# Boese0601/MagicDance

Measured on NVIDIA H100. Metric: denoise-steps/sec @512x512 50-step DDIM, higher is better.
Workload: dtype f16

## Files before the change

### magicdance_b200/csrc/gemm.cu

```cuda
#include <stdlib.h>

#include "common.cuh"

namespace mdb {

constexpr int kBM = 128;
constexpr int kBK = 64;

struct GemmKParams {
  CUtensorMap tmA;
  CUtensorMap tmA2;
  CUtensorMap tmB;
  __half* d;
  long long ldd;
  const float* bias;
  long long bias_batch_stride;
  const __half* residual;
  long long ldr;
  float* ws;
  int rows_per_batch;
  int m, n;
  int k_chunks;
  int k1_chunks;
  int chunks_per_split;
  int splits;
  int conv;
  int chunks_per_tap;
  int w, hw;
  int cs;
  int cluster_reduce;
  const float* ln_u;
  float ln_eps;
};

template <int BN, int STAGES>
struct GemmSmem {
  static constexpr int kABytes = kBM * kBK * 2;
  static constexpr int kBBytes = BN * kBK * 2;
  static constexpr int kStageBytes = kABytes + kBBytes;
  static constexpr int kTotal = STAGES * kStageBytes + 1024;
  static constexpr int kCtasPerSm = (kTotal <= 113 * 1024 && BN <= 128) ? 2 : 1;
};

__device__ __forceinline__ void epi_store_chunk(const GemmKParams& p, long long row, int col0, int ncols,
                                                float (&v)[32], const float* bias_chunk) {
  const __half* rp = (p.residual != nullptr) ? p.residual + row * p.ldr + col0 : nullptr;
  __half* dp = p.d + row * p.ldd + col0;
#pragma unroll
  for (int q = 0; q < 4; ++q) {
    if (q * 8 + 8 <= ncols) {
      float o[8];
#pragma unroll
      for (int e = 0; e < 8; ++e) o[e] = v[q * 8 + e];
      if (bias_chunk != nullptr) {
        const float4 b0 = *reinterpret_cast<const float4*>(bias_chunk + q * 8);
        const float4 b1 = *reinterpret_cast<const float4*>(bias_chunk + q * 8 + 4);
        o[0] += b0.x; o[1] += b0.y; o[2] += b0.z; o[3] += b0.w;
        o[4] += b1.x; o[5] += b1.y; o[6] += b1.z; o[7] += b1.w;
      }
      if (rp != nullptr) {
        const uint4 r4 = *reinterpret_cast<const uint4*>(rp + q * 8);
        const __half2* h2 = reinterpret_cast<const __half2*>(&r4);
#pragma unroll
        for (int e = 0; e < 4; ++e) {
          const float2 f = __half22float2(h2[e]);
          o[2 * e] += f.x;
          o[2 * e + 1] += f.y;
        }
      }
      uint4 o4;
      o4.x = pack_half2(o[0], o[1]);
      o4.y = pack_half2(o[2], o[3]);
      o4.z = pack_half2(o[4], o[5]);
      o4.w = pack_half2(o[6], o[7]);
      *reinterpret_cast<uint4*>(dp + q * 8) = o4;
    } else if (q * 8 < ncols) {
#pragma unroll
      for (int e = 0; e < 8; ++e) {
        const int j = q * 8 + e;
        if (j < ncols) {
          float x = v[j];
          if (bias_chunk != nullptr) x += bias_chunk[j];
          if (rp != nullptr) x += __half2float(rp[j]);
          dp[j] = __float2half_rn(x);
        }
      }
    }
  }
}

template <int BN, bool GEGLU, int kStages>
__global__ void __launch_bounds__(kWsThreads, (GemmSmem<BN, kStages>::kCtasPerSm))
    gemm_tc_kernel(const __grid_constant__ GemmKParams p) {
  using S = GemmSmem<BN, kStages>;
  extern __shared__ uint8_t smem_raw[];
  __shared__ __align__(8) uint64_t full_bar[kStages];
  __shared__ __align__(8) uint64_t empty_bar[kStages];
  __shared__ __align__(16) float s_bias[BN];
  __shared__ __align__(16) float s_lnu[BN];
  __shared__ float2 s_ln[kBM];

  uint8_t* smem = align1024(smem_raw);
  const int warp = threadIdx.x >> 5;
  const int lane = threadIdx.x & 31;
  const int m0 = blockIdx.x * kBM;
  const int n0 = blockIdx.y * BN;
  const int split = blockIdx.z;
  const int kc_begin = split * p.chunks_per_split;
  const int kc_end = min(p.k_chunks, kc_begin + p.chunks_per_split);
  const int n_iter = kc_end - kc_begin;
  constexpr int kRedLd = BN + 4;
  static_assert(kBM * kRedLd * 4 <= kStages * S::kStageBytes, "the accumulator tile must fit in the operand ring");
  const bool ln = p.ln_u != nullptr;

  pdl_launch_dependents();
  if (warp == kProducerWarp && lane == 0) {
    tma_prefetch_desc(&p.tmA);
    tma_prefetch_desc(&p.tmB);
    ring_init<kStages>(full_bar, empty_bar, 1);
    fence_barrier_init();
  }
  const bool bias_in_smem = (p.bias != nullptr) && (p.bias_batch_stride == 0) && !p.cluster_reduce;
  if (bias_in_smem && warp < kProducerWarp) {
    for (int j = threadIdx.x; j < BN; j += kConsumers) s_bias[j] = (n0 + j < p.n) ? p.bias[n0 + j] : 0.f;
  }
  if (ln && warp < kProducerWarp) {
    for (int j = threadIdx.x; j < BN; j += kConsumers) s_lnu[j] = (n0 + j < p.n) ? p.ln_u[n0 + j] : 0.f;
  }
  __syncthreads();
  pdl_wait();

  if (warp == kProducerWarp) {
    if (lane == 0 && n_iter > 0) {
      int b0 = 0, y0 = 0, x0 = 0;
      if (p.conv) {
        b0 = m0 / p.hw;
        y0 = (p.hw >= kBM) ? (m0 % p.hw) / p.w : 0;
        x0 = (p.hw >= kBM) ? (m0 % p.hw) % p.w : 0;
      }
      for (int it = 0; it < n_iter; ++it) {
        const int s = ring_acquire<kStages>(empty_bar, it);
        uint8_t* sa = smem + s * S::kStageBytes;
        uint8_t* sb = sa + S::kABytes;
        const int kc = kc_begin + it;
        mbar_expect_tx(&full_bar[s], S::kStageBytes);
        if (p.conv) {
          const int tap = kc / p.chunks_per_tap;
          const int cc = kc - tap * p.chunks_per_tap;
          const int kh = tap / 3, kw = tap - kh * 3;
          tma_load_4d(sa, &p.tmA, &full_bar[s], cc * kBK, p.cs * x0 + kw - 1, p.cs * y0 + kh - 1, b0);
        } else if (kc < p.k1_chunks) {
          tma_load_2d(sa, &p.tmA, &full_bar[s], kc * kBK, m0);
        } else {
          tma_load_2d(sa, &p.tmA2, &full_bar[s], (kc - p.k1_chunks) * kBK, m0);
        }
        tma_load_2d(sb, &p.tmB, &full_bar[s], kc * kBK, n0);
      }
    }
  } else {
    const int wg = warp >> 2;
    const int tid = threadIdx.x;
    float acc[BN / 2];
#pragma unroll
    for (int i = 0; i < BN / 2; ++i) acc[i] = 0.f;
    const int ln_row = tid >> 1, ln_half = tid & 1;
    float pivot = 0.f, ls0 = 0.f, ls1 = 0.f, lq0 = 0.f, lq1 = 0.f;
    for (int it = 0; it < n_iter; ++it) {
      const int s = ring_wait_full<kStages>(full_bar, it);
      const uint32_t a_addr = smem_u32(smem + s * S::kStageBytes);
      const uint64_t da = wgmma_desc_k_sw128(a_addr + wg * (64 * 128));
      const uint64_t db = wgmma_desc_k_sw128(a_addr + S::kABytes);
      wgmma_fence();
#pragma unroll
      for (int k = 0; k < kBK / 16; ++k) wgmma_ss<BN>(acc, da + 2 * k, db + 2 * k, 1u);
      wgmma_commit();
      if (ln) {
        const uint32_t arow = a_addr + (ln_row >> 3) * 1024 + (ln_row & 7) * 128;
        if (it == 0) {
          uint32_t w0;
          asm volatile("ld.shared.b32 %0, [%1];" : "=r"(w0) : "r"(arow + ((0 ^ (ln_row & 7)) << 4)));
          pivot = __low2float(*reinterpret_cast<const __half2*>(&w0));
        }
#pragma unroll
// ... 57 lines not shown
            if (ch * 32 + j < BN) {
              const float4 f = *reinterpret_cast<const float4*>(rrow + ch * 32 + j);
              v[j] = f.x; v[j + 1] = f.y; v[j + 2] = f.z; v[j + 3] = f.w;
            } else {
              v[j] = v[j + 1] = v[j + 2] = v[j + 3] = 0.f;
            }
          }
          if (ln) {
#pragma unroll
            for (int j = 0; j < 32; ++j)
              if (ch * 32 + j < BN) v[j] = lnst.y * fmaf(-lnst.x, s_lnu[ch * 32 + j], v[j]);
          }
          const int ncols = min(min(32, BN - ch * 32), p.n - col0);
          if (p.splits > 1) {
            if (row_ok) {
              float* wp = p.ws + (static_cast<long long>(split) * p.m + row) * p.n + col0;
#pragma unroll
              for (int j = 0; j < 32; j += 4) {
                if (j + 4 <= ncols && (p.n & 3) == 0) {
                  *reinterpret_cast<float4*>(wp + j) = make_float4(v[j], v[j + 1], v[j + 2], v[j + 3]);
                } else {
#pragma unroll
                  for (int e = 0; e < 4; ++e)
                    if (j + e < ncols) wp[j + e] = v[j + e];
                }
              }
            }
          } else if (row_ok) {
            const float* bias_chunk = nullptr;
            if (bias_in_smem) {
              bias_chunk = s_bias + ch * 32;
            } else if (p.bias != nullptr) {
              const long long brow = (p.bias_batch_stride != 0) ? (row / p.rows_per_batch) : 0;
              bias_chunk = p.bias + brow * p.bias_batch_stride + col0;
            }
            epi_store_chunk(p, row, col0, ncols, v, bias_chunk);
          }
        }
      }
    } else {
      const long long brow = (p.bias_batch_stride != 0) ? (row / p.rows_per_batch) : 0;
#pragma unroll 1
      for (int pr = half; pr < BN / 64; pr += 2) {
        const int col0 = n0 + pr * 64;
        if (col0 >= p.n) break;
        if (row_ok) {
          const float* bp = bias_in_smem ? (s_bias + pr * 64)
                                         : ((p.bias != nullptr) ? p.bias + brow * p.bias_batch_stride + col0 : nullptr);
          const float* rv = rrow + pr * 64;
          uint4* d4 = reinterpret_cast<uint4*>(p.d + row * p.ldd + (col0 >> 1));
#pragma unroll
          for (int q = 0; q < 4; ++q) {
            float o[8];
#pragma unroll
            for (int e = 0; e < 8; ++e) {
              const int j = q * 8 + e;
              float a = rv[j];
              float gt = rv[32 + j];
              if (bp != nullptr) {
                a += bp[j];
                gt += bp[32 + j];
              }
              o[e] = a * gelu_erf_f(gt);
            }
            uint4 o4;
            o4.x = pack_half2(o[0], o[1]);
            o4.y = pack_half2(o[2], o[3]);
            o4.z = pack_half2(o[4], o[5]);
            o4.w = pack_half2(o[6], o[7]);
// ... 18 lines not shown
          const int item = threadIdx.x + q * kWsThreads;
          if (item < R * groups) {
            const int rl = item / groups, cgp = item - rl * groups;
            const long long row = static_cast<long long>(m0) + static_cast<int>(crank) * R + rl;
            const int col0 = n0 + cgp * 8;
            if (row < p.m && col0 + 8 <= p.n) rpre[q] = *reinterpret_cast<const uint4*>(p.residual + row * p.ldr + col0);
          }
        }
      }
      cluster_sync_all();
      const uint32_t red_base = smem_u32(smem);
#pragma unroll 1
      for (int it_ = 0; it_ * kWsThreads < R * groups; ++it_) {
        const int item = threadIdx.x + it_ * kWsThreads;
        if (item >= R * groups) break;
        const int rl = item / groups, cgp = item - rl * groups;
        const int rt = static_cast<int>(crank) * R + rl;
        const long long row = static_cast<long long>(m0) + rt;
        const int col0 = n0 + cgp * 8;
        if (row >= p.m || col0 >= p.n) continue;
        const uint32_t off = red_base + static_cast<uint32_t>((rt * kRedLd + cgp * 8) * 4);
        float o[8];
#pragma unroll
        for (int e = 0; e < 8; ++e) o[e] = 0.f;
        for (int pr = 0; pr < S_; ++pr) {
          const uint32_t ra = dsmem_map(off, static_cast<uint32_t>(pr));
          const float4 a = dsmem_ld_f4(ra), b = dsmem_ld_f4(ra + 16);
          o[0] += a.x; o[1] += a.y; o[2] += a.z; o[3] += a.w;
          o[4] += b.x; o[5] += b.y; o[6] += b.z; o[7] += b.w;
        }
        const int ncols = min(8, p.n - col0);
        const long long brow = (p.bias_batch_stride != 0) ? (row / p.rows_per_batch) : 0;
        if (p.bias != nullptr) {
          const float* bp = p.bias + brow * p.bias_batch_stride + col0;
          for (int e = 0; e < ncols; ++e) o[e] += bp[e];
        }
        if (ncols == 8) {
          if (p.residual != nullptr) {
            uint4 r4 = make_uint4(0, 0, 0, 0);
            if (it_ < kMaxItems) {
#pragma unroll
              for (int q = 0; q < kMaxItems; ++q)
                if (q == it_) r4 = rpre[q];
            } else {
              r4 = *reinterpret_cast<const uint4*>(p.residual + row * p.ldr + col0);
            }
            const __half2* h2 = reinterpret_cast<const __half2*>(&r4);
#pragma unroll
            for (int e = 0; e < 4; ++e) {
              const float2 f = __half22float2(h2[e]);
              o[2 * e] += f.x;
              o[2 * e + 1] += f.y;
            }
          }
          uint4 o4;
          o4.x = pack_half2(o[0], o[1]);
          o4.y = pack_half2(o[2], o[3]);
          o4.z = pack_half2(o[4], o[5]);
          o4.w = pack_half2(o[6], o[7]);
          *reinterpret_cast<uint4*>(p.d + row * p.ldd + col0) = o4;
        } else {
          for (int e = 0; e < ncols; ++e) {
            float x = o[e];
            if (p.residual != nullptr) x += __half2float(p.residual[row * p.ldr + col0 + e]);
            p.d[row * p.ldd + col0 + e] = __float2half_rn(x);
          }
        }
      }
      cluster_sync_all();
    }
  }

}

__global__ void splitk_finalize_kernel(GemmKParams p) {
  pdl_launch_dependents();
  pdl_wait();
  const long long slab = static_cast<long long>(p.m) * p.n;
  if ((p.n & 3) == 0) {
    const long long total4 = slab >> 2;
    for (long long i = static_cast<long long>(blockIdx.x) * blockDim.x + threadIdx.x; i < total4;
         i += static_cast<long long>(gridDim.x) * blockDim.x) {
      const long long e = i << 2;
      const long long row = e / p.n;
      const int col = static_cast<int>(e - row * p.n);
      float4 a = *reinterpret_cast<const float4*>(p.ws + e);
      for (int s = 1; s < p.splits; ++s) {
        const float4 b = *reinterpret_cast<const float4*>(p.ws + s * slab + e);
        a.x += b.x; a.y += b.y; a.z += b.z; a.w += b.w;
      }
      if (p.bias != nullptr) {
        const long long brow = (p.bias_batch_stride != 0) ? (row / p.rows_per_batch) : 0;
        const float* bp = p.bias + brow * p.bias_batch_stride + col;
        a.x += bp[0]; a.y += bp[1]; a.z += bp[2]; a.w += bp[3];
      }
      if (p.residual != nullptr) {
        const __half2* rp = reinterpret_cast<const __half2*>(p.residual + row * p.ldr + col);
        const float2 r0 = __half22float2(rp[0]), r1 = __half22float2(rp[1]);
        a.x += r0.x; a.y += r0.y; a.z += r1.x; a.w += r1.y;
      }
      uint2 o;
      o.x = pack_half2(a.x, a.y);
      o.y = pack_half2(a.z, a.w);
      *reinterpret_cast<uint2*>(p.d + row * p.ldd + col) = o;
    }
    return;
  }
  for (long long i = static_cast<long long>(blockIdx.x) * blockDim.x + threadIdx.x; i < slab;
       i += static_cast<long long>(gridDim.x) * blockDim.x) {
    const long long row = i / p.n;
    const int col = static_cast<int>(i - row * p.n);
    float v = 0.f;
    for (int s = 0; s < p.splits; ++s) v += p.ws[s * slab + i];
    if (p.bias != nullptr) {
      const long long brow = (p.bias_batch_stride != 0) ? (row / p.rows_per_batch) : 0;
      v += p.bias[brow * p.bias_batch_stride + col];
    }
    if (p.residual != nullptr) v += __half2float(p.residual[row * p.ldr + col]);
    p.d[row * p.ldd + col] = __float2half_rn(v);
  }
}

int pixel_box(int ho, int wo, int cs, int rows, bool fwd, uint32_t box[4]) {
  const int hw = ho * wo;
  if (fwd ? wo > rows : wo >= rows) {
    if (wo % rows || (fwd && cs != 1)) return kBoxWideRows;
    box[1] = cs * rows; box[2] = 1; box[3] = 1;
  } else if (hw >= rows) {
    if (rows % wo || hw % rows) return kBoxRowsPerTile;
    box[1] = cs * wo; box[2] = cs * (rows / wo); box[3] = 1;
  } else {
    if (rows % hw) return kBoxImagesPerTile;
    box[1] = cs * wo; box[2] = cs * ho; box[3] = rows / hw;
  }
  box[0] = 64;
  return box[1] <= 256 && box[2] <= 256 ? kBoxOk : kBoxTooLarge;
}

static int g_pair_min_tiles = 128;
static int g_bn80_below = 100;
constexpr int kLongKChunks = 64;

template <int BN, bool GEGLU, int STAGES>
static int launch_gemm(const GemmKParams& kp, dim3 grid, cudaStream_t st) {
  const unsigned cluster_z = kp.cluster_reduce ? static_cast<unsigned>(kp.splits) : 1u;
  constexpr auto kern = gemm_tc_kernel<BN, GEGLU, STAGES>;
  constexpr int kSmem = GemmSmem<BN, STAGES>::kTotal;
  static_assert(kSmem <= 227 * 1024, "shared memory budget");
  if (int rc = set_max_dyn_smem<kern>(kSmem)) return rc;
  MDB_CHECK_CUDA(launch_pdl_cluster(kern, grid, dim3(kWsThreads), kSmem, st, cluster_z, kp));
  count_launch();
  return MDB_OK;
}

int get_gemm_tuning(int key) { return key == MDB_TUNE_GEMM_PAIR_MIN_TILES ? g_pair_min_tiles : g_bn80_below; }
void set_gemm_tuning(int key, int value) {
  if (key == MDB_TUNE_GEMM_PAIR_MIN_TILES) g_pair_min_tiles = value;
  else g_bn80_below = value;
}

}

using namespace mdb;

extern "C" int mdb_gemm_f16(const mdb_gemm_desc* g, mdb_stream_t stream) {
  MDB_REQUIRE(g != nullptr, "mdb_gemm_f16: null descriptor");
  MDB_REQUIRE(g->m > 0 && g->n > 0 && g->k > 0, "mdb_gemm_f16: bad shape m=%d n=%d k=%d", g->m, g->n, g->k);
  MDB_REQUIRE(g->k % kBK == 0, "mdb_gemm_f16: K=%d must be a multiple of 64", g->k);
  MDB_REQUIRE(g->a && g->b && g->d, "mdb_gemm_f16: null operand");
  cudaStream_t st = static_cast<cudaStream_t>(stream);
  const bool geglu = g->epilogue == MDB_EPI_GEGLU;
  GemmKParams kp;
  memset(&kp, 0, sizeof(kp));
  kp.d = static_cast<__half*>(g->d);
  kp.ldd = g->ldd;
  kp.bias = g->bias;
  kp.bias_batch_stride = g->bias_batch_stride;
  kp.rows_per_batch = g->rows_per_batch > 0 ? g->rows_per_batch : 1;
  kp.residual = static_cast<const __half*>(g->residual);
  kp.ldr = g->ldr;
  kp.m = g->m;
  kp.n = g->n;
  kp.k_chunks = g->k / kBK;
  kp.conv = g->conv;
  MDB_REQUIRE(g->ldd % 8 == 0 && (reinterpret_cast<uintptr_t>(g->d) & 15) == 0,
              "mdb_gemm_f16: D must be 16B aligned with ldd %% 8 == 0 (ldd=%lld)", (long long)g->ldd);
  if (g->bias) {
    MDB_REQUIRE((reinterpret_cast<uintptr_t>(g->bias) & 15) == 0 && g->bias_batch_stride % 4 == 0,
                "mdb_gemm_f16: bias must be 16B aligned with bias_batch_stride %% 4 == 0");
  }
  if (g->residual) {
    MDB_REQUIRE(g->ldr % 8 == 0 && (reinterpret_cast<uintptr_t>(g->residual) & 15) == 0,
                "mdb_gemm_f16: residual must be 16B aligned with ldr %% 8 == 0");
    MDB_REQUIRE(!geglu, "mdb_gemm_f16: residual is not supported with the GEGLU epilogue");
  }

  if (g->ln_u != nullptr) {
    MDB_REQUIRE(!geglu, "mdb_gemm_f16: LayerNorm fusion is not available with the GEGLU epilogue (N / 128 CTAs per row "
                        "block would each recompute the row statistics: measured slower than the LayerNorm kernel)");
    MDB_REQUIRE(!g->conv && g->a2 == nullptr && (reinterpret_cast<uintptr_t>(g->ln_u) & 15) == 0,
                "mdb_gemm_f16: LayerNorm fusion needs a plain single-source A whose K is the normalised width");
    kp.ln_u = g->ln_u;
    kp.ln_eps = g->ln_eps;
  }
  int rc;
  if (g->conv) {
    MDB_REQUIRE(g->a2 == nullptr, "mdb_gemm_f16: conv mode takes a single source");
    MDB_REQUIRE(g->c % kBK == 0 && g->k == 9 * g->c, "mdb_gemm_f16: conv needs c %% 64 == 0 and k == 9c (c=%d k=%d)",
                g->c, g->k);
    const int cs = g->conv == 2 ? 2 : 1;
    const int ho = (g->h - 1) / cs + 1, wo = (g->w - 1) / cs + 1;
    MDB_REQUIRE(g->m == g->nb * ho * wo, "mdb_gemm_f16: conv m != nb*ho*wo");
    const int hw = ho * wo;
    uint32_t box[4];
    const int why = pixel_box(ho, wo, cs, kBM, true, box);
    MDB_REQUIRE(why != kBoxWideRows, "mdb_gemm_f16: conv rows wider than 128 pixels need 128 | w and stride 1 (w=%d)", g->w);
    MDB_REQUIRE(why != kBoxRowsPerTile, "mdb_gemm_f16: conv tile needs w | 128 and 128 | h*w (output h=%d w=%d)", ho, wo);
    MDB_REQUIRE(why != kBoxImagesPerTile, "mdb_gemm_f16: conv tile needs h*w | 128 (output h=%d w=%d)", ho, wo);
    MDB_REQUIRE(why != kBoxTooLarge, "mdb_gemm_f16: conv TMA box too large");
    rc = tmap_nhwc(&kp.tmA, g->a, g->c, g->w, g->h, g->nb, g->c, box, cs);
    if (rc) return rc;
    kp.chunks_per_tap = g->c / kBK;
    kp.w = wo;
    kp.hw = hw;
    kp.cs = cs;
    kp.k1_chunks = kp.k_chunks;
  } else {
    const int k1 = g->a2 ? g->k1 : g->k;
    MDB_REQUIRE(k1 % kBK == 0 && k1 > 0 && k1 <= g->k, "mdb_gemm_f16: k1=%d must be a multiple of 64 within K", k1);
    rc = tmap_rows(&kp.tmA, g->a, k1, g->m, g->lda, kBK, kBM);
    if (rc) return rc;
    if (g->a2) {
      rc = tmap_rows(&kp.tmA2, g->a2, g->k - k1, g->m, g->lda2, kBK, kBM);
      if (rc) return rc;
    }
    kp.k1_chunks = k1 / kBK;
  }

  const int m_tiles = (g->m + kBM - 1) / kBM;
  bool pair = g->splits <= 1 && m_tiles >= 2 && g->n % 8 == 0 && g->ln_u == nullptr;
  int bn = 0;
  if (pair) {
    if (geglu) bn = (g->n % 256 == 0) ? 256 : 0;
    else if (g->n % 256 == 0) bn = 256;
    else if (g->n % 160 == 0) bn = 160;
    else bn = 128;
    const long long eq = (long long)m_tiles * ((g->n + bn - 1) / (bn ? bn : 1));
    if (bn == 0 || eq < (long long)g_pair_min_tiles || eq * kp.k_chunks < 16ll * g_pair_min_tiles) pair = false;
  }
  if (pair) {
  } else if (geglu) {
    MDB_REQUIRE(g->n % 128 == 0, "mdb_gemm_f16: GEGLU needs N %% 128 == 0 (N=%d)", g->n);
    bn = 128;
  } else if (g->n % 160 == 0) {
    const long long tiles160 = (long long)m_tiles * (g->n / 160) * (g->splits > 1 ? g->splits : 1);
    const bool wide_split = g->splits == 0 && kp.k_chunks >= kLongKChunks && tiles160 * 2 <= kNumSms;
    bn = (tiles160 < g_bn80_below && !wide_split) ? 80 : 160;
  } else {
    bn = 128;
  }
  rc = tmap_rows(&kp.tmB, g->b, g->k, g->n, g->ldb, kBK, bn);
  if (rc) return rc;

  int splits = g->splits > 1 ? g->splits : 1;
  if (g->ln_u != nullptr) splits = 1;
  if (g->splits == 0 && !geglu && !pair && g->ln_u == nullptr) {
    const long long tiles = (long long)m_tiles * ((g->n + bn - 1) / bn);
    if (tiles < 100)
      for (int c = 8; c >= 2; c >>= 1)
        if (tiles * c <= kNumSms && kp.k_chunks / c >= 16) {
          splits = c;
          break;
        }
  }
  if (splits > kp.k_chunks) splits = kp.k_chunks;
  if (geglu || pair) splits = 1;
  kp.chunks_per_split = (kp.k_chunks + splits - 1) / splits;
  splits = (kp.k_chunks + kp.chunks_per_split - 1) / kp.chunks_per_split;
  kp.splits = splits;
  kp.ws = g->splitk_ws;
  kp.cluster_reduce = (!geglu && (splits == 2 || splits == 4 || splits == 8)) ? 1 : 0;
  if (splits > 1 && !kp.cluster_reduce) {
    MDB_REQUIRE(g->splitk_ws != nullptr, "mdb_gemm_f16: splits > 1 needs splitk_ws");
  }

  dim3 grid(m_tiles, (g->n + bn - 1) / bn, splits);
  const bool deep = (long long)grid.x * grid.y * grid.z <= kNumSms && kp.chunks_per_split >= 12;
// ... 21 lines not shown
```

### magicdance_b200/engine.py

```python
from __future__ import annotations

from dataclasses import dataclass

import torch

from . import ops

UNET = "model.diffusion_model."
APPEARANCE = "appearance_control_model."
POSE = "pose_control_model."


@dataclass(frozen=True)
class NetConfig:
    in_channels: int = 4
    out_channels: int = 4
    hint_channels: int = 3
    model_channels: int = 320
    attention_resolutions: tuple = (4, 2, 1)
    num_res_blocks: int = 2
    channel_mult: tuple = (1, 2, 4, 4)
    num_heads: int = 8
    context_dim: int = 768

# ... 18 lines not shown
            inp.append(blk)
            chans.append(ch)
        if level != len(cfg.channel_mult) - 1:
            inp.append([("down", 0, ch, ch)])
            chans.append(ch)
            ds *= 2
    mid = [("res", 0, ch, ch), ("attn", 1, ch, ch), ("res", 2, ch, ch)]
    out = []
    for level, mult in list(enumerate(cfg.channel_mult))[::-1]:
        for i in range(cfg.num_res_blocks + 1):
            ich = chans.pop()
            blk = [("res", 0, ch + ich, mult * mc)]
            ch = mult * mc
            if ds in cfg.attention_resolutions:
                blk.append(("attn", len(blk), ch, ch))
            if level and i == cfg.num_res_blocks:
                blk.append(("up", len(blk), ch, ch))
                ds //= 2
            out.append(blk)
    return inp, mid, out


def _f16(t, device):
    return t.detach().to(device=device, dtype=torch.float16).contiguous()


def _f32(t, device):
    return t.detach().to(device=device, dtype=torch.float32).contiguous()


def pack_conv3x3(w, device):
    o, i, kh, kw = w.shape
    return _f16(w.detach().to(device).permute(0, 2, 3, 1).reshape(o, kh * kw * i), device)


def pack_conv1x1(w, device):
    return _f16(w.detach().reshape(w.shape[0], w.shape[1]), device)


def pack_geglu(w, b, device):
    n = w.shape[0] // 2
    idx = torch.arange(n).reshape(-1, 32)
    order = torch.cat([idx, idx + n], dim=1).reshape(-1)
    return _f16(w.detach()[order], device), _f32(b.detach()[order], device)


def fold_layernorm(w, gamma, beta, bias, device):
    w, gamma, beta = w.detach().to(device).float(), gamma.detach().to(device).float(), beta.detach().to(device).float()
    w_ln = (w * gamma[None, :]).to(torch.float16).contiguous()
    u = w_ln.float().sum(dim=1).contiguous()
    v = w @ beta
    if bias is not None:
        v = v + bias.detach().to(device).float()
    return w_ln, u, v.contiguous()


class ResW:
    pass


class AttnW:
    pass


class PackedNet:

# ... 8 lines not shown
        emb_w, emb_b, off = [], [], 0
        blocks = [(f"input_blocks.{i}.", b) for i, b in enumerate(self.inp)]
        blocks.append(("middle_block.", self.mid))
        if kind != "controlnet":
            blocks += [(f"output_blocks.{i}.", b) for i, b in enumerate(self.out)]
        for bp, blk in blocks:
            for kind_, j, cin, cout in blk:
                p = f"{bp}{j}."
                if kind_ == "conv_in":
                    self.layers[p] = (pack_conv3x3(g(p + "weight"), device), _f32(g(p + "bias"), device))
                elif kind_ == "res":
                    r = ResW()
                    r.cin, r.cout = cin, cout
                    r.gn1 = (_f32(g(p + "in_layers.0.weight"), device), _f32(g(p + "in_layers.0.bias"), device))
                    r.w1 = pack_conv3x3(g(p + "in_layers.2.weight"), device)
                    r.gn2 = (_f32(g(p + "out_layers.0.weight"), device), _f32(g(p + "out_layers.0.bias"), device))
                    r.w2 = pack_conv3x3(g(p + "out_layers.3.weight"), device)
                    r.b2 = _f32(g(p + "out_layers.3.bias"), device)
                    if (prefix + p + "skip_connection.weight") in sd:
                        r.skip_w = pack_conv1x1(g(p + "skip_connection.weight"), device)
                        r.skip_b = _f32(g(p + "skip_connection.bias"), device)
                    else:
                        r.skip_w = r.skip_b = None
                    emb_w.append(g(p + "emb_layers.1.weight").detach())
                    emb_b.append(g(p + "emb_layers.1.bias").detach() + g(p + "in_layers.2.bias").detach())
                    r.emb_off = off
                    off += cout
                    self.layers[p] = r
                elif kind_ == "attn":
                    self.layers[p] = self._pack_attn(g, p, cin, device)
                elif kind_ == "down":
                    self.layers[p] = (pack_conv3x3(g(p + "op.weight"), device), _f32(g(p + "op.bias"), device))
                elif kind_ == "up":
                    self.layers[p] = (pack_conv3x3(g(p + "conv.weight"), device), _f32(g(p + "conv.bias"), device))
        self.emb_w = _f16(torch.cat(emb_w, 0), device)
        self.emb_b = _f32(torch.cat(emb_b, 0), device)
        self.emb_total = off
        if kind == "unet":
            self.out_gn = (_f32(g("out.0.weight"), device), _f32(g("out.0.bias"), device))
            self.out_w, self.out_b = pack_conv3x3(g("out.2.weight"), device), _f32(g("out.2.bias"), device)
        if kind == "controlnet":
            self.hint = []
            for i in range(8):
                w = g(f"input_hint_block.{2 * i}.weight")
                self.hint.append((pack_conv3x3(w, device), _f32(g(f"input_hint_block.{2 * i}.bias"), device),
                                  w.shape[1], w.shape[0]))
            self.zero = []
            for i in range(len(self.inp)):
                self.zero.append((pack_conv1x1(g(f"zero_convs.{i}.0.weight"), device),
                                  _f32(g(f"zero_convs.{i}.0.bias"), device)))
            self.zero.append((pack_conv1x1(g("middle_block_out.0.weight"), device),
                              _f32(g("middle_block_out.0.bias"), device)))

    def _pack_attn(self, g, p, c, device):
        a = AttnW()
        a.c, a.heads, a.d = c, self.cfg.num_heads, c // self.cfg.num_heads
        a.gn = (_f32(g(p + "norm.weight"), device), _f32(g(p + "norm.bias"), device))
        a.pin_w, a.pin_b = pack_conv1x1(g(p + "proj_in.weight"), device), _f32(g(p + "proj_in.bias"), device)
        a.pout_w, a.pout_b = pack_conv1x1(g(p + "proj_out.weight"), device), _f32(g(p + "proj_out.bias"), device)
        t = p + "transformer_blocks.0."
        for i in (1, 3):
            setattr(a, f"ln{i}", (_f32(g(t + f"norm{i}.weight"), device), _f32(g(t + f"norm{i}.bias"), device)))
        a.wqk = _f16(torch.cat([g(t + "attn1.to_q.weight").detach(), g(t + "attn1.to_k.weight").detach()], 0), device)
        a.wv = _f16(g(t + "attn1.to_v.weight"), device)
        a.wo, a.bo = _f16(g(t + "attn1.to_out.0.weight"), device), _f32(g(t + "attn1.to_out.0.bias"), device)
        a.wq2_ln, a.q2_u, a.q2_v = fold_layernorm(g(t + "attn2.to_q.weight"), g(t + "norm2.weight"), g(t + "norm2.bias"),
                                                  None, device)
# ... 38 lines not shown

_warned_sizes = set()


def _igemm_ok(h, w, c):
    hw = h * w
    if c % 64:
        return False
    ok = ((128 % w == 0 and hw % 128 == 0) or w % 128 == 0) if hw >= 128 else (128 % hw == 0)
    if not ok and (h, w) not in _warned_sizes:
        _warned_sizes.add((h, w))
        import warnings
        warnings.warn(f"magicdance_b200: a {h}x{w} feature map does not tile into 128-pixel TMA boxes; its 3x3 convs take "
                      "the slower im2col + GEMM path (latents whose width divides 128 avoid this)", stacklevel=3)
    return ok


def conv3x3(x: Act, w, bias, *, cout, stride=1, residual=None, bias_batch_stride=0) -> Act:
    cin = x.c
    ho, wo = (x.h - 1) // stride + 1, (x.w - 1) // stride + 1
    tc = cout % 8 == 0 and cout >= 64 and cin % 64 == 0
    if tc and _igemm_ok(ho, wo, cin):
        y = ops.gemm(x.data, w, bias=bias, bias_batch_stride=bias_batch_stride, rows_per_batch=ho * wo,
                     residual=residual, conv=(x.b, x.h, x.w, cin), conv_stride=stride)
    elif tc:
        col = ops.im2col3x3(x.data, batch=x.b, h=x.h, w=x.w, c=cin, stride=stride)
        y = ops.gemm(col, w, bias=bias, bias_batch_stride=bias_batch_stride, rows_per_batch=ho * wo,
                     residual=residual)
    else:
        assert bias_batch_stride == 0
        y = ops.conv3x3_direct(x.data, w, bias, batch=x.b, h=x.h, w=x.w, cin=cin, cout=cout, stride=stride,
                               residual=residual)
    return Act(y, x.b, ho, wo)


class _BankComplete(Exception):
    """unwinds appearance_write as soon as the last norm1 state is in the bank"""


class DenoiseEngine:

    def __init__(self, state_dict, cfg: NetConfig | None = None, device="cuda"):
        ops.ensure_device()
        self.cfg = cfg or NetConfig()
        self.device = torch.device(device)
        self.unet = PackedNet(state_dict, UNET, self.cfg, "unet", self.device)
        self.appearance = PackedNet(state_dict, APPEARANCE, self.cfg, "appearance", self.device)
        self.pose = PackedNet(state_dict, POSE, self.cfg, "controlnet", self.device)
        self._ctx_cache = {}

    @classmethod
    def from_packed(cls, unet: "PackedNet", appearance: "PackedNet | None", pose: "PackedNet | None"):
        ops.ensure_device()
        self = cls.__new__(cls)
        first = unet or appearance or pose
        self.cfg, self.device = first.cfg, first.device
        self.unet, self.appearance, self.pose = unet, appearance, pose
        self._ctx_cache = {}
        return self

    def time_bias(self, net: PackedNet, t: torch.Tensor, rows=None):
        if t.shape[0] == 1:
            rows = 1
        e = ops.timestep_embedding(t, self.cfg.model_channels, rows)
        e = ops.skinny_linear(e, net.te0_w, net.te0_b, silu_out=True)
        e = ops.skinny_linear(e, net.te2_w, net.te2_b)
# ... 65 lines not shown
            k1, vt1, nb1, kvb1 = bank_kv
            kw = dict(k1=k1, vt1=vt1, n1=nb1, kv1_batches=kvb1, bank_batches=min(bank_batches, b))
        at = ops.attention(qk[:, :c], qk[:, c:], vt, n, heads=a.heads, d=a.d, batch=b, nq=n, **kw)
        h = ops.gemm(at, a.wo, bias=a.bo, residual=h)
        q2 = ops.gemm(h, a.wq2_ln, bias=a.q2_v, ln_u=a.q2_u, ln_eps=1e-5)
        kt, vtt, nt, kvb, ldv = ctx_kv
        at2 = ops.attention(q2, kt, vtt, nt, heads=a.heads, d=a.d, batch=b, nq=n, kv0_batches=kvb if kvb == b else 1,
                            ldv0_batch=ldv)
        h = ops.gemm(at2, a.wo2, bias=a.bo2, residual=h)
        n3 = ops.layernorm(h, *a.ln3)
        ff = ops.gemm(n3, a.wff1, bias=a.bff1, epilogue=ops.EPI_GEGLU)
        h = ops.gemm(ff, a.wff2, bias=a.bff2, residual=h)
        y = ops.gemm(h, a.pout_w, bias=a.pout_b, residual=x.data)
        return Act(y, x.b, x.h, x.w)

    def _run_block(self, net, bp, blk, x: Act, skip, emb_all, ctx_kvs, state):
        for kind, j, cin, cout in blk:
            p = f"{bp}{j}."
            lw = net.layers[p]
            if kind == "conv_in":
                x = conv3x3(x, lw[0], lw[1], cout=cout, residual=state.get("hint"))
            elif kind == "res":
                x = self._res(lw, x, skip, emb_all)
                skip = None
            elif kind == "attn":
                i = state["attn_i"]
                bank_kv = state["bank_kv"][i] if state.get("bank_kv") is not None else None
                x = self._transformer(lw, x, ctx_kvs[i], state["mode"], state.get("bank"), bank_kv,
                                      state.get("bank_batches", 0))
                state["attn_i"] = i + 1
            elif kind == "down":
                x = conv3x3(x, lw[0], lw[1], cout=cout, stride=2)
            elif kind == "up":
                up = ops.upsample2x(x.data, batch=x.b, h=x.h, w=x.w, c=x.c)
                x = conv3x3(Act(up, x.b, 2 * x.h, 2 * x.w), lw[0], lw[1], cout=cout)
        return x

    def _prep(self, x_nchw, context, copies=1):
        x = x_nchw.to(device=self.device, dtype=torch.float32)
        b, c, h, w = x.shape
        act = Act(ops.nchw_f32_to_nhwc_f16(x, copies=copies), copies * b, h, w)
        ctx16 = context.to(device=self.device, dtype=torch.float16).contiguous()
        return act, ctx16

    def appearance_write(self, ref_latent, t, context):
        net = self.appearance
        x, ctx16 = self._prep(ref_latent, context)
        ctx_kvs = self.context_kv(net, ctx16, context)
        emb_all = self.time_bias(net, t, x.b)
        n_total = len(net.attn_layers())
        state = {"mode": "write", "attn_i": 0, "bank": [], "bank_batches": n_total}
        hs = []
        try:
            for i, blk in enumerate(net.inp):
                x = self._run_block(net, f"input_blocks.{i}.", blk, x, None, emb_all, ctx_kvs, state)
                hs.append(x)
            x = self._run_block(net, "middle_block.", net.mid, x, None, emb_all, ctx_kvs, state)
            for i, blk in enumerate(net.out):
                x = self._run_block(net, f"output_blocks.{i}.", blk, x, hs.pop(), emb_all, ctx_kvs, state)
        except _BankComplete:
            pass
        return state["bank"]

    def attn_geometry(self, h, w):
        net = self.unet
        geo = []
        for blk in net.inp:
            for kind, _, _, cout in blk:
# ... 134 lines not shown
```

### magicdance_b200/ops.py

```python
from __future__ import annotations

import ctypes as C
import os

import torch

from . import _lib

EPI_NONE, EPI_GEGLU = 0, 1
SKINNY_MAX_ROWS = 16
_GEMM_DEBUG = os.environ.get("MDB_GEMM_DEBUG", "0") == "1"
TRACE = None


class tuning:
    _KEYS = {"pair_min_tiles": _lib.TUNE_GEMM_PAIR_MIN_TILES,
             "attn40_2q_min_ctas": _lib.TUNE_ATTN40_2Q_MIN_CTAS, "bn80_below": _lib.TUNE_GEMM_BN80_BELOW}

    def __init__(self, **kw):
        self.want = {self._KEYS[k]: int(v) for k, v in kw.items() if v is not None}

    def __enter__(self):
        lib = _lib.load()
        self.old = {k: int(lib.mdb_get_tuning(k)) for k in self.want}
        for k, v in self.want.items():
            _lib.check(lib.mdb_set_tuning(k, v), "set_tuning")
        return self

    def __exit__(self, *a):
        lib = _lib.load()
        for k, v in self.old.items():
            lib.mdb_set_tuning(k, v)


def _stream() -> int:
    return torch.cuda.current_stream().cuda_stream


def _ptr(t):
    return None if t is None else t.data_ptr()


# ... 35 lines not shown

    def __enter__(self):
        global _ws_tag
        self.prev, _ws_tag = _ws_tag, self.tag

    def __exit__(self, *a):
        global _ws_tag
        _ws_tag = self.prev


def current_lane():
    return _ws_tag


_ws_retired = []


def _workspace(key, numel, dtype, device, zero=False):
    k = (key, device, _ws_tag)
    t = _ws_cache.get(k)
    if t is None or t.numel() < numel or t.dtype != dtype:
        if t is not None:
            _ws_retired.append(t)
            numel = max(numel, 2 * t.numel())
        alloc = torch.zeros if zero else torch.empty
        t = alloc(max(numel, 1), dtype=dtype, device=device)
        _ws_cache[k] = t
    return t


def _gemm_m(a, conv, conv_stride, m):
    if conv is not None:
        nb, h, wd, _ = conv
        return nb * ((h - 1) // conv_stride + 1) * ((wd - 1) // conv_stride + 1)
    return a.shape[0] if m is None else m


def _fill_fwd_desc(g, a, w, a2, conv, conv_stride, m):
    n, k = w.shape
    if conv is not None:
        nb, h, wd, c = conv
        assert conv_stride in (1, 2) and a.is_contiguous() and a.numel() == nb * h * wd * c
        g.conv, g.nb, g.h, g.w, g.c = conv_stride, nb, h, wd, c
        g.a, g.lda, g.k1 = a.data_ptr(), c, k
    else:
        assert a.dim() == 2 and a.stride(1) == 1
        g.a, g.lda, g.k1 = a.data_ptr(), a.stride(0), a.shape[1]
        if a2 is not None:
            _chk(a2, torch.float16, "a2")
            assert a2.dim() == 2 and a2.stride(1) == 1 and a2.shape[0] == a.shape[0]
            g.a2, g.lda2 = a2.data_ptr(), a2.stride(0)
            assert a.shape[1] + a2.shape[1] == k
        else:
            assert a.shape[1] == k, (a.shape, w.shape)
    m = _gemm_m(a, conv, conv_stride, m)
    g.m, g.n, g.k = m, n, k
    return m, g.k1


def gemm(a, w, *, out=None, bias=None, bias_batch_stride=0, rows_per_batch=0, residual=None, epilogue=EPI_NONE,
         a2=None, conv=None, conv_stride=1, splits=0, m=None, ln_u=None, ln_eps=1e-5):
    lib = _lib.load()
    _chk(a, torch.float16, "a")
    _chk(w, torch.float16, "w")
    g = _lib.GemmDesc()
    n, k = w.shape
    m, _ = _fill_fwd_desc(g, a, w, a2, conv, conv_stride, m)
    n_out = n // 2 if epilogue == EPI_GEGLU else n
    if out is None:
        out = torch.empty((m, n_out), dtype=torch.float16, device=a.device)
    _chk(out, torch.float16, "out")
    assert out.dim() == 2 and out.stride(1) == 1 and out.shape[0] >= m and out.shape[1] == n_out, (out.shape, m, n_out)
    assert w.stride(1) == 1
    g.b, g.ldb = w.data_ptr(), w.stride(0)
    g.d, g.ldd = out.data_ptr(), out.stride(0)
    if bias is not None:
        _chk(bias, torch.float32, "bias")
        g.bias, g.bias_batch_stride, g.rows_per_batch = bias.data_ptr(), bias_batch_stride, rows_per_batch
    if residual is not None:
        _chk(residual, torch.float16, "residual")
        assert residual.dim() == 2 and residual.stride(1) == 1
        g.residual, g.ldr = residual.data_ptr(), residual.stride(0)
    g.epilogue = epilogue
    if ln_u is not None:
        _chk(ln_u, torch.float32, "ln_u")
        assert conv is None and a2 is None and ln_u.numel() == n and ln_u.is_contiguous()
        g.ln_u, g.ln_eps = ln_u.data_ptr(), float(ln_eps)
        splits = 1
    if TRACE is not None:
        TRACE.append((m, n, k, (tuple(conv) + (conv_stride,)) if conv is not None else None, epilogue, splits,
                      a2.shape[1] if a2 is not None else 0))
    if splits > 1:
        ws = _workspace("splitk", splits * m * n, torch.float32, a.device)
        g.splits, g.splitk_ws = splits, ws.data_ptr()
    else:
        g.splits = splits
    if _GEMM_DEBUG:
        import sys
        print(f"gemm m={m} n={n} k={k} conv={conv} epi={epilogue} splits={g.splits} a2={a2 is not None} lda={g.lda} "
              f"ldd={g.ldd} bias={bias is not None} bbs={g.bias_batch_stride} res={residual is not None}",
              file=sys.stderr, flush=True)
    _lib.check(lib.mdb_gemm_f16(C.byref(g), _stream()), "gemm_f16")
    if _GEMM_DEBUG:
        torch.cuda.synchronize()
    return out
# ... 757 lines not shown
```

Baseline: 89.92.

## Fuse nearest-2x upsample into the following 3x3 conv via four 2x2 phase convs

Replaces the separate upsample2x kernel plus a 3x3 conv on the upsampled map with a single implicit-GEMM over the low-resolution input. The weights are pre-summed into four 2x2 phase kernels, stacked along N. The epilogue scatters each phase's columns to the interleaved high-resolution output rows. This removes the upsampled intermediate's memory traffic and cuts the reduction length from 9c to 4c per output pixel. In exchange it adds per-element address arithmetic in the epilogue, strided output writes, and fp16 rounding of the summed weights.

```diff
diff --git a/magicdance_b200/csrc/gemm.cu b/magicdance_b200/csrc/gemm.cu
--- a/magicdance_b200/csrc/gemm.cu
+++ b/magicdance_b200/csrc/gemm.cu
@@ -28,6 +28,7 @@
   int chunks_per_tap;
   int w, hw;
   int cs;
+  int up_n;
   int cluster_reduce;
   const float* ln_u;
   float ln_eps;
@@ -42,10 +43,24 @@
   static constexpr int kCtasPerSm = (kTotal <= 113 * 1024 && BN <= 128) ? 2 : 1;
 };
 
+template <bool UP>
+__device__ __forceinline__ __half* d_at(const GemmKParams& p, long long row, int col) {
+  if (!UP) return p.d + row * p.ldd + col;
+  const int ph = col / p.up_n;
+  const long long img = row / p.hw;
+  const int r = static_cast<int>(row - img * p.hw);
+  const int y = r / p.w, x = r - y * p.w;
+  const long long orow = (img * (2 * (p.hw / p.w)) + 2 * y + (ph >> 1)) * (2 * p.w) + 2 * x + (ph & 1);
+  return p.d + orow * p.ldd + (col - ph * p.up_n);
+}
+template <bool UP>
+__device__ __forceinline__ int bias_col(const GemmKParams& p, int col) { return UP ? col % p.up_n : col; }
+
+template <bool UP>
 __device__ __forceinline__ void epi_store_chunk(const GemmKParams& p, long long row, int col0, int ncols,
                                                 float (&v)[32], const float* bias_chunk) {
   const __half* rp = (p.residual != nullptr) ? p.residual + row * p.ldr + col0 : nullptr;
-  __half* dp = p.d + row * p.ldd + col0;
+  __half* dp = d_at<UP>(p, row, col0);
 #pragma unroll
   for (int q = 0; q < 4; ++q) {
     if (q * 8 + 8 <= ncols) {
@@ -89,7 +104,7 @@
   }
 }
 
-template <int BN, bool GEGLU, int kStages>
+template <int BN, bool GEGLU, int kStages, bool UP>
 __global__ void __launch_bounds__(kWsThreads, (GemmSmem<BN, kStages>::kCtasPerSm))
     gemm_tc_kernel(const __grid_constant__ GemmKParams p) {
   using S = GemmSmem<BN, kStages>;
@@ -109,6 +124,9 @@
   const int kc_begin = split * p.chunks_per_split;
   const int kc_end = min(p.k_chunks, kc_begin + p.chunks_per_split);
   const int n_iter = kc_end - kc_begin;
+  const int phase = UP ? n0 / p.up_n : 0;
+  const int py = phase >> 1, px = phase & 1;
+  constexpr int kTaps = UP ? 2 : 3;
   constexpr int kRedLd = BN + 4;
   static_assert(kBM * kRedLd * 4 <= kStages * S::kStageBytes, "the accumulator tile must fit in the operand ring");
   const bool ln = p.ln_u != nullptr;
@@ -122,7 +140,7 @@
   }
   const bool bias_in_smem = (p.bias != nullptr) && (p.bias_batch_stride == 0) && !p.cluster_reduce;
   if (bias_in_smem && warp < kProducerWarp) {
-    for (int j = threadIdx.x; j < BN; j += kConsumers) s_bias[j] = (n0 + j < p.n) ? p.bias[n0 + j] : 0.f;
+    for (int j = threadIdx.x; j < BN; j += kConsumers) s_bias[j] = (n0 + j < p.n) ? p.bias[bias_col<UP>(p, n0 + j)] : 0.f;
   }
   if (ln && warp < kProducerWarp) {
     for (int j = threadIdx.x; j < BN; j += kConsumers) s_lnu[j] = (n0 + j < p.n) ? p.ln_u[n0 + j] : 0.f;
@@ -147,8 +165,8 @@
         if (p.conv) {
           const int tap = kc / p.chunks_per_tap;
           const int cc = kc - tap * p.chunks_per_tap;
-          const int kh = tap / 3, kw = tap - kh * 3;
-          tma_load_4d(sa, &p.tmA, &full_bar[s], cc * kBK, p.cs * x0 + kw - 1, p.cs * y0 + kh - 1, b0);
+          const int kh = tap / kTaps, kw = tap - kh * kTaps;
+          tma_load_4d(sa, &p.tmA, &full_bar[s], cc * kBK, p.cs * x0 + kw + px - 1, p.cs * y0 + kh + py - 1, b0);
         } else if (kc < p.k1_chunks) {
           tma_load_2d(sa, &p.tmA, &full_bar[s], kc * kBK, m0);
         } else {
@@ -272,9 +290,9 @@
               bias_chunk = s_bias + ch * 32;
             } else if (p.bias != nullptr) {
               const long long brow = (p.bias_batch_stride != 0) ? (row / p.rows_per_batch) : 0;
-              bias_chunk = p.bias + brow * p.bias_batch_stride + col0;
+              bias_chunk = p.bias + brow * p.bias_batch_stride + bias_col<UP>(p, col0);
             }
-            epi_store_chunk(p, row, col0, ncols, v, bias_chunk);
+            epi_store_chunk<UP>(p, row, col0, ncols, v, bias_chunk);
           }
         }
       }
@@ -359,7 +377,7 @@
         const int ncols = min(8, p.n - col0);
         const long long brow = (p.bias_batch_stride != 0) ? (row / p.rows_per_batch) : 0;
         if (p.bias != nullptr) {
-          const float* bp = p.bias + brow * p.bias_batch_stride + col0;
+          const float* bp = p.bias + brow * p.bias_batch_stride + bias_col<UP>(p, col0);
           for (int e = 0; e < ncols; ++e) o[e] += bp[e];
         }
         if (ncols == 8) {
@@ -385,12 +403,13 @@
           o4.y = pack_half2(o[2], o[3]);
           o4.z = pack_half2(o[4], o[5]);
           o4.w = pack_half2(o[6], o[7]);
-          *reinterpret_cast<uint4*>(p.d + row * p.ldd + col0) = o4;
+          *reinterpret_cast<uint4*>(d_at<UP>(p, row, col0)) = o4;
         } else {
+          __half* dp = d_at<UP>(p, row, col0);
           for (int e = 0; e < ncols; ++e) {
             float x = o[e];
             if (p.residual != nullptr) x += __half2float(p.residual[row * p.ldr + col0 + e]);
-            p.d[row * p.ldd + col0 + e] = __float2half_rn(x);
+            dp[e] = __float2half_rn(x);
           }
         }
       }
@@ -418,7 +437,7 @@
       }
       if (p.bias != nullptr) {
         const long long brow = (p.bias_batch_stride != 0) ? (row / p.rows_per_batch) : 0;
-        const float* bp = p.bias + brow * p.bias_batch_stride + col;
+        const float* bp = p.bias + brow * p.bias_batch_stride + (p.up_n ? bias_col<true>(p, col) : col);
         a.x += bp[0]; a.y += bp[1]; a.z += bp[2]; a.w += bp[3];
       }
       if (p.residual != nullptr) {
@@ -429,7 +448,7 @@
       uint2 o;
       o.x = pack_half2(a.x, a.y);
       o.y = pack_half2(a.z, a.w);
-      *reinterpret_cast<uint2*>(p.d + row * p.ldd + col) = o;
+      *reinterpret_cast<uint2*>(p.up_n ? d_at<true>(p, row, col) : d_at<false>(p, row, col)) = o;
     }
     return;
   }
@@ -441,10 +460,10 @@
     for (int s = 0; s < p.splits; ++s) v += p.ws[s * slab + i];
     if (p.bias != nullptr) {
       const long long brow = (p.bias_batch_stride != 0) ? (row / p.rows_per_batch) : 0;
-      v += p.bias[brow * p.bias_batch_stride + col];
+      v += p.bias[brow * p.bias_batch_stride + (p.up_n ? bias_col<true>(p, col) : col)];
     }
     if (p.residual != nullptr) v += __half2float(p.residual[row * p.ldr + col]);
-    p.d[row * p.ldd + col] = __float2half_rn(v);
+    *(p.up_n ? d_at<true>(p, row, col) : d_at<false>(p, row, col)) = __float2half_rn(v);
   }
 }
 
@@ -468,16 +487,24 @@
 static int g_bn80_below = 100;
 constexpr int kLongKChunks = 64;
 
-template <int BN, bool GEGLU, int STAGES>
-static int launch_gemm(const GemmKParams& kp, dim3 grid, cudaStream_t st) {
+template <int BN, bool GEGLU, int STAGES, bool UP>
+static int launch_gemm_t(const GemmKParams& kp, dim3 grid, cudaStream_t st) {
   const unsigned cluster_z = kp.cluster_reduce ? static_cast<unsigned>(kp.splits) : 1u;
-  constexpr auto kern = gemm_tc_kernel<BN, GEGLU, STAGES>;
+  constexpr auto kern = gemm_tc_kernel<BN, GEGLU, STAGES, UP>;
   constexpr int kSmem = GemmSmem<BN, STAGES>::kTotal;
   static_assert(kSmem <= 227 * 1024, "shared memory budget");
   if (int rc = set_max_dyn_smem<kern>(kSmem)) return rc;
   MDB_CHECK_CUDA(launch_pdl_cluster(kern, grid, dim3(kWsThreads), kSmem, st, cluster_z, kp));
   count_launch();
   return MDB_OK;
+}
+
+template <int BN, bool GEGLU, int STAGES>
+static int launch_gemm(const GemmKParams& kp, dim3 grid, cudaStream_t st) {
+  if constexpr (!GEGLU) {
+    if (kp.up_n) return launch_gemm_t<BN, false, STAGES, true>(kp, grid, st);
+  }
+  return launch_gemm_t<BN, GEGLU, STAGES, false>(kp, grid, st);
 }
 
 int get_gemm_tuning(int key) { return key == MDB_TUNE_GEMM_PAIR_MIN_TILES ? g_pair_min_tiles : g_bn80_below; }
@@ -531,10 +558,21 @@
     kp.ln_eps = g->ln_eps;
   }
   int rc;
+  const bool up = g->conv == 3;
   if (g->conv) {
     MDB_REQUIRE(g->a2 == nullptr, "mdb_gemm_f16: conv mode takes a single source");
-    MDB_REQUIRE(g->c % kBK == 0 && g->k == 9 * g->c, "mdb_gemm_f16: conv needs c %% 64 == 0 and k == 9c (c=%d k=%d)",
+    const int taps = up ? 2 : 3;
+    MDB_REQUIRE(g->c % kBK == 0 && g->k == taps * taps * g->c,
+                "mdb_gemm_f16: conv needs c %% 64 == 0 and k == 9c (4c for the phase convs of an Upsample) (c=%d k=%d)",
                 g->c, g->k);
+    if (up) {
+      kp.up_n = g->n / 4;
+      MDB_REQUIRE(g->n % 4 == 0 && (kp.up_n % 128 == 0 || kp.up_n % 160 == 0),
+                  "mdb_gemm_f16: an Upsample's phase convs need N = 4 * cout with cout %% 128 == 0 or %% 160 == 0 (N=%d)",
+                  g->n);
+      MDB_REQUIRE(!geglu && g->residual == nullptr && g->bias_batch_stride == 0,
+                  "mdb_gemm_f16: an Upsample's phase convs take a plain bias only (no residual, per-batch bias, GEGLU)");
+    }
     const int cs = g->conv == 2 ? 2 : 1;
     const int ho = (g->h - 1) / cs + 1, wo = (g->w - 1) / cs + 1;
     MDB_REQUIRE(g->m == g->nb * ho * wo, "mdb_gemm_f16: conv m != nb*ho*wo");
@@ -565,12 +603,13 @@
   }
 
   const int m_tiles = (g->m + kBM - 1) / kBM;
+  const int nq = up ? kp.up_n : g->n;
   bool pair = g->splits <= 1 && m_tiles >= 2 && g->n % 8 == 0 && g->ln_u == nullptr;
   int bn = 0;
   if (pair) {
     if (geglu) bn = (g->n % 256 == 0) ? 256 : 0;
-    else if (g->n % 256 == 0) bn = 256;
-    else if (g->n % 160 == 0) bn = 160;
+    else if (nq % 256 == 0) bn = 256;
+    else if (nq % 160 == 0) bn = 160;
     else bn = 128;
     const long long eq = (long long)m_tiles * ((g->n + bn - 1) / (bn ? bn : 1));
     if (bn == 0 || eq < (long long)g_pair_min_tiles || eq * kp.k_chunks < 16ll * g_pair_min_tiles) pair = false;
@@ -579,7 +618,7 @@
   } else if (geglu) {
     MDB_REQUIRE(g->n % 128 == 0, "mdb_gemm_f16: GEGLU needs N %% 128 == 0 (N=%d)", g->n);
     bn = 128;
-  } else if (g->n % 160 == 0) {
+  } else if (nq % 160 == 0) {
     const long long tiles160 = (long long)m_tiles * (g->n / 160) * (g->splits > 1 ? g->splits : 1);
     const bool wide_split = g->splits == 0 && kp.k_chunks >= kLongKChunks && tiles160 * 2 <= kNumSms;
     bn = (tiles160 < g_bn80_below && !wide_split) ? 80 : 160;
diff --git a/magicdance_b200/engine.py b/magicdance_b200/engine.py
--- a/magicdance_b200/engine.py
+++ b/magicdance_b200/engine.py
@@ -74,6 +74,21 @@
 def pack_conv3x3(w, device):
     o, i, kh, kw = w.shape
     return _f16(w.detach().to(device).permute(0, 2, 3, 1).reshape(o, kh * kw * i), device)
+
+
+def pack_upconv(w, device):
+    wf = w.detach().to(device).float()
+    taps = {(0, 0): (0,), (0, 1): (1, 2), (1, 0): (0, 1), (1, 1): (2,)}
+    o, i = wf.shape[:2]
+    out = torch.zeros((4, o, 2, 2, i), dtype=torch.float32, device=device)
+    for py in (0, 1):
+        for px in (0, 1):
+            for dy in (0, 1):
+                for dx in (0, 1):
+                    for kh in taps[(py, dy)]:
+                        for kw in taps[(px, dx)]:
+                            out[2 * py + px, :, dy, dx, :] += wf[:, :, kh, kw]
+    return out.reshape(4 * o, 4 * i).to(torch.float16).contiguous()
 
 
 def pack_conv1x1(w, device):
@@ -148,7 +163,8 @@
                 elif kind_ == "down":
                     self.layers[p] = (pack_conv3x3(g(p + "op.weight"), device), _f32(g(p + "op.bias"), device))
                 elif kind_ == "up":
-                    self.layers[p] = (pack_conv3x3(g(p + "conv.weight"), device), _f32(g(p + "conv.bias"), device))
+                    self.layers[p] = (pack_conv3x3(g(p + "conv.weight"), device), _f32(g(p + "conv.bias"), device),
+                                      pack_upconv(g(p + "conv.weight"), device))
         self.emb_w = _f16(torch.cat(emb_w, 0), device)
         self.emb_b = _f32(torch.cat(emb_b, 0), device)
         self.emb_total = off
@@ -253,6 +269,18 @@
         y = ops.conv3x3_direct(x.data, w, bias, batch=x.b, h=x.h, w=x.w, cin=cin, cout=cout, stride=stride,
                                residual=residual)
     return Act(y, x.b, ho, wo)
+
+
+UPCONV_MIN_PIXELS = 4096
+
+
+def upsample_conv3x3(x: Act, lw, *, cout) -> Act:
+    if (x.data.is_cuda and x.b * x.h * x.w >= UPCONV_MIN_PIXELS and (cout % 128 == 0 or cout % 160 == 0)
+            and _igemm_ok(x.h, x.w, x.c)):
+        y = ops.gemm(x.data, lw[2], bias=lw[1], conv=(x.b, x.h, x.w, x.c), conv_stride=ops.UPSAMPLE2X)
+        return Act(y, x.b, 2 * x.h, 2 * x.w)
+    up = ops.upsample2x(x.data, batch=x.b, h=x.h, w=x.w, c=x.c)
+    return conv3x3(Act(up, x.b, 2 * x.h, 2 * x.w), lw[0], lw[1], cout=cout)
 
 
 class _BankComplete(Exception):
@@ -384,8 +412,7 @@
             elif kind == "down":
                 x = conv3x3(x, lw[0], lw[1], cout=cout, stride=2)
             elif kind == "up":
-                up = ops.upsample2x(x.data, batch=x.b, h=x.h, w=x.w, c=x.c)
-                x = conv3x3(Act(up, x.b, 2 * x.h, 2 * x.w), lw[0], lw[1], cout=cout)
+                x = upsample_conv3x3(x, lw, cout=cout)
         return x
 
     def _prep(self, x_nchw, context, copies=1):
diff --git a/magicdance_b200/ops.py b/magicdance_b200/ops.py
--- a/magicdance_b200/ops.py
+++ b/magicdance_b200/ops.py
@@ -8,6 +8,7 @@
 from . import _lib
 
 EPI_NONE, EPI_GEGLU = 0, 1
+UPSAMPLE2X = 3
 SKINNY_MAX_ROWS = 16
 _GEMM_DEBUG = os.environ.get("MDB_GEMM_DEBUG", "0") == "1"
 TRACE = None
@@ -109,7 +110,8 @@
 def _gemm_m(a, conv, conv_stride, m):
     if conv is not None:
         nb, h, wd, _ = conv
-        return nb * ((h - 1) // conv_stride + 1) * ((wd - 1) // conv_stride + 1)
+        s = 1 if conv_stride == UPSAMPLE2X else conv_stride
+        return nb * ((h - 1) // s + 1) * ((wd - 1) // s + 1)
     return a.shape[0] if m is None else m
 
 
@@ -117,7 +119,7 @@
     n, k = w.shape
     if conv is not None:
         nb, h, wd, c = conv
-        assert conv_stride in (1, 2) and a.is_contiguous() and a.numel() == nb * h * wd * c
+        assert conv_stride in (1, 2, UPSAMPLE2X) and a.is_contiguous() and a.numel() == nb * h * wd * c
         g.conv, g.nb, g.h, g.w, g.c = conv_stride, nb, h, wd, c
         g.a, g.lda, g.k1 = a.data_ptr(), c, k
     else:
@@ -143,11 +145,14 @@
     g = _lib.GemmDesc()
     n, k = w.shape
     m, _ = _fill_fwd_desc(g, a, w, a2, conv, conv_stride, m)
-    n_out = n // 2 if epilogue == EPI_GEGLU else n
+    up = conv is not None and conv_stride == UPSAMPLE2X
+    n_out = n // 2 if epilogue == EPI_GEGLU else (n // 4 if up else n)
+    m_out = 4 * m if up else m
     if out is None:
-        out = torch.empty((m, n_out), dtype=torch.float16, device=a.device)
+        out = torch.empty((m_out, n_out), dtype=torch.float16, device=a.device)
     _chk(out, torch.float16, "out")
-    assert out.dim() == 2 and out.stride(1) == 1 and out.shape[0] >= m and out.shape[1] == n_out, (out.shape, m, n_out)
+    assert out.dim() == 2 and out.stride(1) == 1 and out.shape[0] >= m_out and out.shape[1] == n_out, (out.shape, m_out,
+                                                                                                        n_out)
     assert w.stride(1) == 1
     g.b, g.ldb = w.data_ptr(), w.stride(0)
     g.d, g.ldd = out.data_ptr(), out.stride(0)
```

New measurement: 90.49 (median of 6 runs). About the same (+0.6%).
